# lschoenm/MerKurio

Measured on AMD Instinct MI355X. Metric: Gbases/s scanned (150bp FASTQ, 10k 31-mers); % HBM roofline at 1/2/4/8 GPUs, higher is better.
Workload: dtype u8

## Files before the change

### merkurio_amd/csrc/codec/bgzf_inflate_wave.hip

```cpp
#include <hip/hip_runtime.h>

#include "codec_kernels.h"
#include "inflate_wave_common.hpp"

namespace mkz {

namespace {

template <uint32_t kRing>
struct WaveLds {
    uint8_t ring[kRing];
    uint16_t ll_fast[1 << kFastLl];
    uint32_t d_fast[1 << kFastD];
    uint16_t ll_limit[16], ll_base[16], d_limit[16], d_base[16];
    uint16_t ll_sorted[288], d_sorted[32];
    uint8_t lens[320];
};
static_assert(sizeof(WaveLds<32768>) <= 40 * 1024, "four waves per CU");
static_assert(sizeof(WaveLds<8192>) <= 14 * 1024, "eleven waves per CU");
static_assert(sizeof(WaveLds<4096>) <= 9728, "seventeen waves per CU");

}

template <uint32_t kRing>
__global__ __launch_bounds__(64) void mk_bgzf_inflate_wave_kernel(const uint8_t *__restrict__ in_all, uint64_t n_in_all, const Member *__restrict__ members,
                                                                  uint32_t n_members, uint8_t *__restrict__ out_all, int32_t *__restrict__ status_out) {
    constexpr uint32_t kFlush = kRing >= 8192 ? 4096u : kRing / 2;
    static_assert(kRing >= 2 * kFlush && kFlush >= 1024 && (kRing & (kRing - 1)) == 0, "ring: a power of two that holds two flush pieces");
    constexpr uint32_t kRingMask = kRing - 1;
    extern __shared__ uint8_t lds_raw[];
    WaveLds<kRing> &S = *reinterpret_cast<WaveLds<kRing> *>(lds_raw);
    const uint32_t lane = lane_id();
    const uint32_t mi = blockIdx.x;
    if (mi >= n_members) return;
    const Member m = members[mi];
    const uint8_t *in = in_all + m.data_off;
    const uint32_t n_in = m.data_len, n_out = m.isize;
    uint8_t *const out = out_all + m.out_off;

    uint32_t s0 = 0, sbase = 0, rd = 0;
    uint32_t look = 0, nxt = 0;
    uint64_t bitbuf = 0;
    uint32_t bitcnt = 0;
    auto load_dword = [&](uint32_t dw) -> uint32_t {
        const uint32_t byte = s0 + 4 * dw;
        return byte <= n_in + 8 ? load_le32(in + byte) : 0u;
    };
    auto restart = [&](uint32_t byte_pos) {
        s0 = byte_pos, sbase = 0, rd = 0, bitbuf = 0, bitcnt = 0;
        look = load_dword(lane);
        nxt = load_dword(64 + lane);
    };
#define MKW_NEED32()                                                                              \
    do {                                                                                          \
        if (bitcnt < 32) {                                                                        \
            uint32_t k_ = uni(rd - sbase);                                                        \
            if (k_ == 64) {                                                                       \
                look = nxt, sbase += 64, k_ = 0;                                                  \
                nxt = load_dword(sbase + 64 + lane);                                              \
            }                                                                                     \
            bitbuf |= (uint64_t)(uint32_t)__builtin_amdgcn_readlane((int)look, (int)k_) << bitcnt; \
            bitcnt += 32, ++rd;                                                                   \
        }                                                                                         \
    } while (0)
#define MKW_TAKE(n) (bitbuf >>= (n), bitcnt -= (n))
#define MKW_TAKEN() (s0 + 4 * rd)
#define MKW_RAN_OUT() (MKW_TAKEN() > n_in + 8)
    restart(0);

    uint32_t op = 0, flushed = 0;
    int status = 0;
    auto flush_blocks = [&]() {
        while (op - flushed >= kFlush) {
#pragma unroll
            for (uint32_t k = 0; k < kFlush; k += 1024) {
                const uint32_t at = flushed + k + 16 * lane;
                const uint4 v = *reinterpret_cast<const uint4 *>(&S.ring[at & kRingMask]);
                __builtin_memcpy(out + at, &v, 16);
            }
            flushed += kFlush;
        }
        if (kRing < 32768) {
            __builtin_amdgcn_fence(__ATOMIC_RELEASE, "workgroup");
            __builtin_amdgcn_s_waitcnt(0x0F70);
        }
    };

    for (bool last_block = false; !last_block && status == 0;) {
        MKW_NEED32();
        if (MKW_RAN_OUT()) {
            status = kInfTruncated;
            break;
        }
        last_block = ((uint32_t)bitbuf & 1u) != 0;
        const uint32_t type = ((uint32_t)bitbuf >> 1) & 3u;
        MKW_TAKE(3);
        if (type == 3) {
            status = kInfBadBlockType;
            break;
        }
        if (type == 0) {
            MKW_TAKE(bitcnt & 7);
            MKW_NEED32();
            const uint32_t len = (uint32_t)bitbuf & 0xffffu, nlen = ((uint32_t)(bitbuf >> 16)) & 0xffffu;
            MKW_TAKE(32);
            const uint32_t pos = MKW_TAKEN() - (bitcnt >> 3);
            if ((len ^ nlen) != 0xffffu) status = kInfBadStored;
            else if (MKW_RAN_OUT() || pos > n_in || len > n_in - pos) status = kInfTruncated;
            else if (len > n_out - op) status = kInfOutputOverrun;
            if (status) break;
            for (uint32_t done = 0; done < len;) {
                const uint32_t piece = min(len - done, kFlush);
                for (uint32_t i = lane; i < piece; i += 64) S.ring[(op + i) & kRingMask] = in[pos + done + i];
                op += piece, done += piece;
                flush_blocks();
            }
            restart(pos + len);
            continue;
        }
        if (type == 1) {
            for (uint32_t i = lane; i < 320; i += 64) S.lens[i] = (uint8_t)(i < 144 ? 8 : i < 256 ? 9 : i < 280 ? 7 : i < 288 ? 8 : 5);
        } else {
            const uint32_t hlit = ((uint32_t)bitbuf & 31u) + 257, hdist = ((uint32_t)(bitbuf >> 5) & 31u) + 1, hclen = ((uint32_t)(bitbuf >> 10) & 15u) + 4;
            MKW_TAKE(14);
            if (hlit > 286 || hdist > 30) {
                status = kInfBadLengths;
                break;
            }
            if (lane < (uint32_t)kCl) S.lens[lane] = 0;
            constexpr uint64_t kOrderLo = 16ull | 17ull << 5 | 18ull << 10 | 0ull << 15 | 8ull << 20 | 7ull << 25 | 9ull << 30 | 6ull << 35 | 10ull << 40 |
                                          5ull << 45 | 11ull << 50 | 4ull << 55;
            constexpr uint64_t kOrderHi = 12ull | 3ull << 5 | 13ull << 10 | 2ull << 15 | 14ull << 20 | 1ull << 25 | 15ull << 30;
            for (uint32_t i = 0; i < hclen; ++i) {
                MKW_NEED32();
                const uint32_t sym = (uint32_t)((i < 12 ? kOrderLo >> (5 * i) : kOrderHi >> (5 * (i - 12))) & 31u);
                if (lane == 0) S.lens[sym] = (uint8_t)((uint32_t)bitbuf & 7u);
                MKW_TAKE(3);
            }
            if (wave_build_tables(S.lens, kCl, S.ll_sorted, S.ll_limit, S.ll_base, false)) {
                status = kInfBadLengths;
                break;
            }
            uint32_t i = 0, prev_len = 0;
            while (i < hlit + hdist && status == 0) {
                MKW_NEED32();
                if (MKW_RAN_OUT()) {
                    status = kInfTruncated;
                    break;
                }
                const uint32_t e = decode_codeword((uint32_t)bitbuf, S.ll_sorted, S.ll_limit, S.ll_base);
                if (e == 0 || (e & 15u) > (uint32_t)kMaxClBits) {
                    status = kInfBadLengths;
                    break;
                }
                MKW_TAKE(e & 15u);
                const uint32_t sym = e >> 4;
                if (sym < 16) {
                    if (lane == 0) S.lens[i < hlit ? i : 288 + (i - hlit)] = (uint8_t)sym;
                    prev_len = sym, ++i;
                    continue;
                }
                uint32_t rep, val = 0;
                if (sym == 16) {
                    if (i == 0) {
                        status = kInfBadLengths;
                        break;
                    }
                    val = prev_len;
                    rep = 3 + ((uint32_t)bitbuf & 3u);
                    MKW_TAKE(2);
                } else if (sym == 17) {
                    rep = 3 + ((uint32_t)bitbuf & 7u);
                    MKW_TAKE(3);
                } else {
                    rep = 11 + ((uint32_t)bitbuf & 127u);
                    MKW_TAKE(7);
                }
                if (i + rep > hlit + hdist) {
                    status = kInfBadLengths;
                    break;
                }
                if (lane < rep) {
                    const uint32_t j = i + lane;
                    S.lens[j < hlit ? j : 288 + (j - hlit)] = (uint8_t)val;
                }
                if (lane + 64 < rep) {
                    const uint32_t j = i + lane + 64;
                    S.lens[j < hlit ? j : 288 + (j - hlit)] = (uint8_t)val;
                }
                if (lane + 128 < rep) {
                    const uint32_t j = i + lane + 128;
                    S.lens[j < hlit ? j : 288 + (j - hlit)] = (uint8_t)val;
                }
                prev_len = val, i += rep;
            }
            if (status) break;
            for (uint32_t k = hlit + lane; k < 288; k += 64) S.lens[k] = 0;
            if (lane + hdist < 32) S.lens[288 + hdist + lane] = 0;
            __builtin_amdgcn_wave_barrier();
            if (S.lens[256] == 0) {
                status = kInfBadLengths;
                break;
            }
        }
        __builtin_amdgcn_wave_barrier();
        if (wave_build_tables(S.lens, 288, S.ll_sorted, S.ll_limit, S.ll_base, true) ||
            wave_build_tables(S.lens + 288, type == 1 ? 32 : 30, S.d_sorted, S.d_limit, S.d_base, true)) {
            status = kInfBadLengths;
            break;
        }
        __builtin_amdgcn_wave_barrier();
        wave_fill_fast_ll(S.ll_fast, S.ll_sorted, S.ll_limit, S.ll_base);
        wave_fill_fast_d(S.d_fast, S.d_sorted, S.d_limit, S.d_base);
        __builtin_amdgcn_wave_barrier();

        uint32_t flush_at = flushed + kFlush;
        for (;;) {
            MKW_NEED32();
            uint32_t e = S.ll_fast[(uint32_t)bitbuf & ((1u << kFastLl) - 1)];
            if (e == 0) {
                e = pack_ll(decode_codeword((uint32_t)bitbuf, S.ll_sorted, S.ll_limit, S.ll_base));
                if (e == 0) {
                    status = kInfBadSymbol;
                    break;
                }
            }
            MKW_TAKE(e & 15u);
            if (e < 0x1000u) {
                S.ring[op & kRingMask] = (uint8_t)(e >> 4);
                ++op;
                if (op < flush_at) continue;
            } else if (e < 0x8000u) {
                break;
            } else {
                const uint32_t leb = (e >> 4) & 7u;
                const uint32_t len = ((e >> 7) & 255u) + 3u + ((uint32_t)bitbuf & ((1u << leb) - 1));
                MKW_TAKE(leb);
                MKW_NEED32();
                uint32_t d = S.d_fast[(uint32_t)bitbuf & ((1u << kFastD) - 1)];
                if (d == 0) {
                    d = pack_d(decode_codeword((uint32_t)bitbuf, S.d_sorted, S.d_limit, S.d_base));
                    if (d == 0) {
                        status = kInfBadSymbol;
                        break;
                    }
                }
                MKW_TAKE(d & 15u);
                const uint32_t deb = (d >> 4) & 15u;
                const uint32_t dist = (d >> 8) + ((uint32_t)bitbuf & ((1u << deb) - 1));
                MKW_TAKE(deb);
                if (dist > op) {
                    status = kInfBadDistance;
                    break;
                }
                const uint32_t src0 = op - dist;
                if (kRing < 32768 && dist + len > kRing) {
                    for (uint32_t i = lane; i < len; i += 64) {
                        const uint32_t p = src0 + i;
                        const uint8_t b = p < flushed ? __hip_atomic_load(out + p, __ATOMIC_RELAXED, __HIP_MEMORY_SCOPE_AGENT) : S.ring[p & kRingMask];
                        S.ring[(op + i) & kRingMask] = b;
                    }
                } else if (dist >= len) {
                    for (uint32_t i = lane; i < len; i += 64) S.ring[(op + i) & kRingMask] = S.ring[(src0 + i) & kRingMask];
                } else {
                    for (uint32_t i = lane; i < len; i += 64) S.ring[(op + i) & kRingMask] = S.ring[(src0 + i % dist) & kRingMask];
                }
                op += len;
                if (op < flush_at) continue;
            }
            if (op > n_out) {
                status = kInfOutputOverrun;
                break;
            }
            if (MKW_RAN_OUT()) {
                status = kInfTruncated;
                break;
            }
            flush_blocks();
            flush_at = flushed + kFlush;
        }
        if (status == 0 && op > n_out) status = kInfOutputOverrun;
        if (status == 0 && MKW_RAN_OUT()) status = kInfTruncated;
    }
    if (status == 0 && (MKW_RAN_OUT() || (uint64_t)MKW_TAKEN() - (bitcnt >> 3) > (uint64_t)n_in)) status = kInfTruncated;
    if (status == 0 && op != n_out) status = kInfOutputShort;
    if (status == 0) {
        flush_blocks();
        for (uint32_t i = flushed + lane; i < op; i += 64) out[i] = S.ring[i & kRingMask];
    }
    if (lane == 0) status_out[mi] = status;
#undef MKW_NEED32
#undef MKW_TAKE
#undef MKW_TAKEN
#undef MKW_RAN_OUT
}

template <uint32_t kRing>
static void launch_ring(const uint8_t *in, uint64_t n_in, const Member *members, uint32_t n_members, uint8_t *out, int32_t *status, hipStream_t s) {
    static bool raised = false;
    if (!raised) {
        (void)hipFuncSetAttribute((const void *)mk_bgzf_inflate_wave_kernel<kRing>, hipFuncAttributeMaxDynamicSharedMemorySize, (int)sizeof(WaveLds<kRing>));
        raised = true;
    }
    hipLaunchKernelGGL(mk_bgzf_inflate_wave_kernel<kRing>, dim3(n_members), dim3(64), sizeof(WaveLds<kRing>), s, in, n_in, members, n_members, out, status);
}

void launch_inflate_wave(const uint8_t *in, uint64_t n_in, const Member *members, uint32_t n_members, uint8_t *out, int32_t *status, hipStream_t s,
                         uint32_t ring_bytes) {
    if (!n_members) return;
    if (ring_bytes == 2048) launch_ring<2048>(in, n_in, members, n_members, out, status, s);
    else if (ring_bytes == 4096) launch_ring<4096>(in, n_in, members, n_members, out, status, s);
    else if (ring_bytes == 8192) launch_ring<8192>(in, n_in, members, n_members, out, status, s);
    else if (ring_bytes == 16384) launch_ring<16384>(in, n_in, members, n_members, out, status, s);
    else launch_ring<32768>(in, n_in, members, n_members, out, status, s);
}

}
```

### merkurio_amd/csrc/codec/gzip_segments_wave.hpp

```cpp
#pragma once
#include <hip/hip_runtime.h>

#include <type_traits>

#include "gzip_segments.hpp"
#include "inflate_wave_common.hpp"

namespace mkz {
namespace {

#ifndef MK_SEG_PAIRS
#define MK_SEG_PAIRS 0
#endif
constexpr bool kSegPairs = MK_SEG_PAIRS != 0;
#ifndef MK_SEG_RING
#define MK_SEG_RING 2048
#endif
constexpr uint32_t kSegRing = MK_SEG_RING, kSegRingMask = kSegRing - 1, kSegFlush = kSegRing / 2;
constexpr uint64_t kSegCapMax = 0xfff00000ull;
constexpr int kSegCutShort = 1;
constexpr uint64_t kSegConfirmSymbols = 2048;

struct SegWaveTables {
    std::conditional_t<kSegPairs, uint32_t, uint16_t> ll_fast[1 << kFastLl];
    uint32_t d_fast[1 << kFastD];
    uint16_t ll_limit[16], ll_base[16], d_limit[16], d_base[16];
    uint16_t ll_sorted[288], d_sorted[32];
    uint8_t lens[320];
};
static_assert(kSegRing != 2048 || sizeof(SegWaveTables) + 2 * kSegRing <= (kSegPairs ? 11648 : 9728), "fourteen (without pairs: seventeen) waves per CU");
static_assert(kSegRing >= 1024 && (kSegRing & (kSegRing - 1)) == 0, "the flush writes 512 symbols a step");

template <bool kDry>
__device__ __forceinline__ int wave_inflate_segment(const uint8_t *__restrict__ in, uint64_t n_in, uint64_t bit0, uint64_t bit_end, uint32_t max_blocks,
                                    uint16_t *__restrict__ out, uint64_t cap, uint16_t *ring, SegWaveTables &S, uint64_t max_symbols, uint64_t *n_out,
                                    uint64_t *bit_stop, bool *final_seen) {
    const uint32_t lane = lane_id();
    uint64_t s0 = 0;
    uint32_t sbase = 0, rd = 0;
    uint32_t look = 0, nxt = 0;
    uint64_t bitbuf = 0;
    uint32_t bitcnt = 0;
    auto load_dword = [&](uint32_t dw) -> uint32_t {
        const uint64_t byte = s0 + 4ull * dw;
        return byte <= n_in + 8 ? load_le32(in + byte) : 0u;
    };
    auto restart = [&](uint64_t byte_pos) {
        s0 = byte_pos, sbase = 0, rd = 0, bitbuf = 0, bitcnt = 0;
        look = load_dword(lane);
        nxt = load_dword(64 + lane);
    };
#define MKS_NEED32()                                                                              \
    do {                                                                                          \
        if (bitcnt < 32) {                                                                        \
            uint32_t k_ = uni(rd - sbase);                                                        \
            if (k_ == 64) {                                                                       \
                look = nxt, sbase += 64, k_ = 0;                                                  \
                nxt = load_dword(sbase + 64 + lane);                                              \
            }                                                                                     \
            bitbuf |= (uint64_t)(uint32_t)__builtin_amdgcn_readlane((int)look, (int)k_) << bitcnt; \
            bitcnt += 32, ++rd;                                                                   \
        }                                                                                         \
    } while (0)
#define MKS_TAKE(n) (bitbuf >>= (n), bitcnt -= (n))
#define MKS_BITPOS() ((s0 + 4ull * rd) * 8 - bitcnt)
#define MKS_RAN_OUT() (MKS_BITPOS() > n_in * 8)
    restart(bit0 >> 3);
    MKS_NEED32();
    MKS_TAKE((uint32_t)bit0 & 7u);

    uint32_t op = 0, flushed = 0;
    const uint32_t cap32 = (uint32_t)(cap < kSegCapMax ? cap : kSegCapMax);
    int status = 0;
    bool fin = false;
    auto flush_blocks = [&]() {
        while (op - flushed >= kSegFlush) {
            if constexpr (!kDry) {
#pragma unroll
                for (uint32_t k = 0; k < kSegFlush; k += 512) {
                    const uint32_t at = flushed + k + 8 * lane;
                    const uint4 v = *reinterpret_cast<const uint4 *>(&ring[at & kSegRingMask]);
                    __builtin_memcpy(out + at, &v, 16);
                }
            }
            flushed += kSegFlush;
        }
        if constexpr (!kDry) {
            __builtin_amdgcn_fence(__ATOMIC_RELEASE, "workgroup");
            __builtin_amdgcn_s_waitcnt(0x0F70);
        }
    };

    for (uint32_t blocks = 0;; ++blocks) {
        const uint64_t at = MKS_BITPOS();
        if (at == bit_end || (max_blocks && blocks == max_blocks)) break;
        if (at > bit_end) {
            status = kSegDesync;
            break;
        }
        MKS_NEED32();
        if (MKS_RAN_OUT()) {
            status = kInfTruncated;
            break;
        }
        const bool final_block = ((uint32_t)bitbuf & 1u) != 0;
        const uint32_t type = ((uint32_t)bitbuf >> 1) & 3u;
        MKS_TAKE(3);
        if (type == 3) {
            status = kInfBadBlockType;
            break;
        }
        if (type == 0) {
            MKS_TAKE(bitcnt & 7);
            MKS_NEED32();
            const uint32_t len = (uint32_t)bitbuf & 0xffffu, nlen = ((uint32_t)(bitbuf >> 16)) & 0xffffu;
            MKS_TAKE(32);
            const uint64_t pos = MKS_BITPOS() >> 3;
            if ((len ^ nlen) != 0xffffu) status = kInfBadStored;
            else if (MKS_RAN_OUT() || pos > n_in || len > n_in - pos) status = kInfTruncated;
            else if (len > cap32 - op) status = kSegOverflow;
            if (status) break;
            for (uint32_t done = 0; done < len;) {
                const uint32_t piece = min(len - done, kSegFlush);
                if constexpr (!kDry)
                    for (uint32_t i = lane; i < piece; i += 64) ring[(op + i) & kSegRingMask] = in[pos + done + i];
                op += piece, done += piece;
                flush_blocks();
            }
            restart(pos + len);
        } else {
            if (type == 1) {
                for (uint32_t i = lane; i < 320; i += 64) S.lens[i] = (uint8_t)(i < 144 ? 8 : i < 256 ? 9 : i < 280 ? 7 : i < 288 ? 8 : 5);
            } else {
                const uint32_t hlit = ((uint32_t)bitbuf & 31u) + 257, hdist = ((uint32_t)(bitbuf >> 5) & 31u) + 1, hclen = ((uint32_t)(bitbuf >> 10) & 15u) + 4;
                MKS_TAKE(14);
                if (hlit > 286 || hdist > 30) {
                    status = kInfBadLengths;
                    break;
                }
                if (lane < (uint32_t)kCl) S.lens[lane] = 0;
                constexpr uint64_t kOrderLo = 16ull | 17ull << 5 | 18ull << 10 | 0ull << 15 | 8ull << 20 | 7ull << 25 | 9ull << 30 | 6ull << 35 | 10ull << 40 |
                                              5ull << 45 | 11ull << 50 | 4ull << 55;
                constexpr uint64_t kOrderHi = 12ull | 3ull << 5 | 13ull << 10 | 2ull << 15 | 14ull << 20 | 1ull << 25 | 15ull << 30;
                for (uint32_t i = 0; i < hclen; ++i) {
                    MKS_NEED32();
                    const uint32_t s_ = (uint32_t)((i < 12 ? kOrderLo >> (5 * i) : kOrderHi >> (5 * (i - 12))) & 31u);
                    if (lane == 0) S.lens[s_] = (uint8_t)((uint32_t)bitbuf & 7u);
                    MKS_TAKE(3);
                }
                if (wave_build_tables(S.lens, kCl, S.ll_sorted, S.ll_limit, S.ll_base, false)) {
                    status = kInfBadLengths;
                    break;
                }
                uint32_t i = 0, prev_len = 0;
                while (i < hlit + hdist && status == 0) {
                    MKS_NEED32();
                    if (MKS_RAN_OUT()) {
                        status = kInfTruncated;
                        break;
                    }
                    const uint32_t e = decode_codeword((uint32_t)bitbuf, S.ll_sorted, S.ll_limit, S.ll_base);
                    if (e == 0 || (e & 15u) > (uint32_t)kMaxClBits) {
                        status = kInfBadLengths;
                        break;
                    }
                    MKS_TAKE(e & 15u);
                    const uint32_t cs = e >> 4;
                    if (cs < 16) {
                        if (lane == 0) S.lens[i < hlit ? i : 288 + (i - hlit)] = (uint8_t)cs;
                        prev_len = cs, ++i;
                        continue;
                    }
                    uint32_t rep, val = 0;
                    if (cs == 16) {
                        if (i == 0) {
                            status = kInfBadLengths;
                            break;
                        }
                        val = prev_len;
                        rep = 3 + ((uint32_t)bitbuf & 3u);
                        MKS_TAKE(2);
                    } else if (cs == 17) {
                        rep = 3 + ((uint32_t)bitbuf & 7u);
                        MKS_TAKE(3);
                    } else {
                        rep = 11 + ((uint32_t)bitbuf & 127u);
                        MKS_TAKE(7);
                    }
                    if (i + rep > hlit + hdist) {
                        status = kInfBadLengths;
                        break;
                    }
                    for (uint32_t q = lane; q < rep; q += 64) {
                        const uint32_t x = i + q;
                        S.lens[x < hlit ? x : 288 + (x - hlit)] = (uint8_t)val;
                    }
                    prev_len = val, i += rep;
                }
                if (status) break;
                for (uint32_t k = hlit + lane; k < 288; k += 64) S.lens[k] = 0;
                if (lane + hdist < 32) S.lens[288 + hdist + lane] = 0;
                __builtin_amdgcn_wave_barrier();
                if (S.lens[256] == 0) {
                    status = kInfBadLengths;
                    break;
                }
            }
            __builtin_amdgcn_wave_barrier();
            if (wave_build_tables(S.lens, 288, S.ll_sorted, S.ll_limit, S.ll_base, true) ||
                wave_build_tables(S.lens + 288, type == 1 ? 32 : 30, S.d_sorted, S.d_limit, S.d_base, true)) {
                status = kInfBadLengths;
                break;
            }
            __builtin_amdgcn_wave_barrier();
            for (uint32_t e = lane; e < (1u << kFastLl); e += 64) {
                const uint32_t r = decode_codeword(e, S.ll_sorted, S.ll_limit, S.ll_base);
                S.ll_fast[e] = (r & 15u) <= (uint32_t)kFastLl ? pack_ll(r) : 0u;
            }
            __builtin_amdgcn_wave_barrier();
            if constexpr (kSegPairs) {
                for (uint32_t e = lane; e < (1u << kFastLl); e += 64) {
                    const uint32_t a = reinterpret_cast<const uint16_t *>(S.ll_fast)[2 * e];
                    const uint32_t la = a & 15u;
                    if (a != 0 && a < 0x1000u && la < (uint32_t)kFastLl) {
                        const uint32_t b = reinterpret_cast<const uint16_t *>(S.ll_fast)[2 * (e >> la)];
                        if (b != 0 && b < 0x1000u && la + (b & 15u) <= (uint32_t)kFastLl) reinterpret_cast<uint16_t *>(S.ll_fast)[2 * e + 1] = (uint16_t)((b & 0xff0u) | (la + (b & 15u)));
                    }
                }
            }
            wave_fill_fast_d(S.d_fast, S.d_sorted, S.d_limit, S.d_base);
            __builtin_amdgcn_wave_barrier();

            uint32_t flush_at = flushed + kSegFlush;
            for (;;) {
                MKS_NEED32();
                uint32_t e = S.ll_fast[(uint32_t)bitbuf & ((1u << kFastLl) - 1)];
                if (kSegPairs && e > 0xffffu) {
                    if constexpr (!kDry) {
                        ring[op & kSegRingMask] = (uint16_t)((e >> 4) & 0xffu);
                        ring[(op + 1) & kSegRingMask] = (uint16_t)(e >> 20);
                    }
                    MKS_TAKE((e >> 16) & 15u);
                    op += 2;
                    if (op < flush_at) continue;
                    e = 0x10000u;
                } else if (e == 0) {
                    e = pack_ll(decode_codeword((uint32_t)bitbuf, S.ll_sorted, S.ll_limit, S.ll_base));
                    if (e == 0) {
                        status = kInfBadSymbol;
                        break;
                    }
                }
                if (e != 0x10000u) {
                    MKS_TAKE(e & 15u);
                    if (e < 0x1000u) {
                        if constexpr (!kDry) ring[op & kSegRingMask] = (uint16_t)(e >> 4);
                        ++op;
                        if (op < flush_at) continue;
                    } else if (e < 0x8000u) {
                        break;
                    } else {
                        const uint32_t leb = (e >> 4) & 7u;
                        const uint32_t len = ((e >> 7) & 255u) + 3u + ((uint32_t)bitbuf & ((1u << leb) - 1));
                        MKS_TAKE(leb);
                        MKS_NEED32();
                        uint32_t d = S.d_fast[(uint32_t)bitbuf & ((1u << kFastD) - 1)];
                        if (d == 0) {
                            d = pack_d(decode_codeword((uint32_t)bitbuf, S.d_sorted, S.d_limit, S.d_base));
                            if (d == 0) {
                                status = kInfBadSymbol;
                                break;
                            }
                        }
                        MKS_TAKE(d & 15u);
                        const uint32_t deb = (d >> 4) & 15u;
                        const uint32_t dist = (d >> 8) + ((uint32_t)bitbuf & ((1u << deb) - 1));
                        MKS_TAKE(deb);
                        if constexpr (!kDry) {
                            const uint32_t src0 = op - dist;
                            if (dist + len > kSegRing || dist > op) {
                                for (uint32_t i = lane; i < len; i += 64) {
                                    const long long p = (long long)op - (long long)dist + (dist >= len ? i : i % dist);
                                    const uint16_t v = p < (long long)flushed ? __hip_atomic_load(out + p, __ATOMIC_RELAXED, __HIP_MEMORY_SCOPE_AGENT)
                                                                               : ring[(uint64_t)p & kSegRingMask];
                                    ring[(op + i) & kSegRingMask] = v;
                                }
                            } else if (dist >= len) {
                                for (uint32_t i = lane; i < len; i += 64) ring[(op + i) & kSegRingMask] = ring[(src0 + i) & kSegRingMask];
                            } else {
                                for (uint32_t i = lane; i < len; i += 64) ring[(op + i) & kSegRingMask] = ring[(src0 + i % dist) & kSegRingMask];
                            }
                        }
                        op += len;
                        if (op < flush_at) continue;
                    }
                }
                if (op > cap32) {
                    status = kSegOverflow;
                    break;
                }
                if (MKS_RAN_OUT()) {
                    status = kInfTruncated;
                    break;
                }
                if constexpr (kDry) {
                    if (max_symbols && op >= max_symbols) {
                        status = kSegCutShort;
                        break;
                    }
                }
                flush_blocks();
                flush_at = flushed + kSegFlush;
            }
            if (status == 0 && op > cap32) status = kSegOverflow;
            if (status == 0 && MKS_RAN_OUT()) status = kInfTruncated;
            if (status) break;
        }
        if (final_block) {
            fin = true;
            break;
        }
    }
    if constexpr (!kDry) {
        if (status == 0) {
            flush_blocks();
            for (uint32_t i = flushed + lane; i < op; i += 64) out[i] = ring[i & kSegRingMask];
        }
    }
    *n_out = op;
    *bit_stop = MKS_BITPOS();
    *final_seen = fin;
    return status;
#undef MKS_NEED32
#undef MKS_TAKE
#undef MKS_BITPOS
#undef MKS_RAN_OUT
}

__device__ __forceinline__ bool wave_confirm_block_start(const uint8_t *__restrict__ in, uint64_t n_in, uint64_t bit, SegWaveTables &S) {
    uint64_t n_out = 0, stop = 0;
    bool fin = false;
    const int rc = wave_inflate_segment<true>(in, n_in, bit, ~0ull, 1, nullptr, ~0ull, nullptr, S, kSegConfirmSymbols, &n_out, &stop, &fin);
    if (rc == kSegCutShort) return true;
    if (rc != 0) return false;
    if (n_out == 0 || fin) return false;
    if (stop + 3 > n_in * 8) return false;
    SegReader r;
    r.in = in, r.n_in = n_in;
    sr_seek(r, stop);
    const uint32_t type = ((uint32_t)r.bitbuf >> 1) & 3u;
    if (type == 2) {
        sr_take(r, 3);
        return seg_dynamic_header(r, nullptr) == 0;
    }
    if (type == 0) {
        sr_take(r, 3);
        sr_take(r, r.bitcnt & 7);
        sr_need32(r);
        const uint32_t len = (uint32_t)r.bitbuf & 0xffffu, nlen = ((uint32_t)(r.bitbuf >> 16)) & 0xffffu;
        return (len ^ nlen) == 0xffffu;
    }
    return false;
}

}
}
```

### merkurio_amd/csrc/codec/inflate_wave_common.hpp

```cpp
#pragma once
#include <hip/hip_runtime.h>

#include "inflate_serial.hpp"

namespace mkz {
namespace {

constexpr int kFastLl = 10, kFastD = 9;

__device__ __forceinline__ uint32_t lane_id() { return __builtin_amdgcn_mbcnt_hi(~0u, __builtin_amdgcn_mbcnt_lo(~0u, 0u)); }
__device__ __forceinline__ uint32_t uni(uint32_t v) { return (uint32_t)__builtin_amdgcn_readfirstlane((int)v); }

__device__ int wave_build_tables(const uint8_t *lens, uint32_t n, uint16_t *sorted, uint16_t *limit, uint16_t *base, bool allow_single) {
    const uint32_t lane = lane_id();
    uint32_t cnt = 0, used = 0;
    for (uint32_t i = 0; i < n; ++i) {
        const uint32_t v = lens[i];
        cnt += (v == lane);
        used += (v != 0);
    }
    if (lane == 0 || lane > (uint32_t)kMaxBits) cnt = 0;
    int left = 1;
    uint32_t code = 0, off = 0, my_off = 0, prev = 0;
    bool over = false;
    if (lane == 0) limit[0] = 0, base[0] = 0;
    for (uint32_t l = 1; l <= (uint32_t)kMaxBits; ++l) {
        const uint32_t c = (uint32_t)__builtin_amdgcn_readlane((int)cnt, (int)l);
        left = (left << 1) - (int)c;
        over = over || left < 0;
        code = (code + prev) << 1;
        if (lane == l) {
            my_off = off;
            limit[l] = (uint16_t)((code + c) << (kMaxBits - l));
            base[l] = (uint16_t)(off - code);
        }
        off += c;
        prev = c;
    }
    if (over) return 1;
    for (uint32_t c0 = 0; c0 < n; c0 += 64) {
        const uint32_t i = c0 + lane;
        const uint32_t mine = i < n ? lens[i] : 0u;
        for (uint32_t l = 1; l <= (uint32_t)kMaxBits; ++l) {
            const uint64_t m = __ballot(mine == l);
            if (m == 0) continue;
            const uint32_t o = (uint32_t)__builtin_amdgcn_readlane((int)my_off, (int)l);
            if (mine == l) sorted[o + (uint32_t)__popcll(m & ((1ull << lane) - 1))] = (uint16_t)i;
            if (lane == l) my_off += (uint32_t)__popcll(m);
        }
    }
    const uint32_t c1 = (uint32_t)__builtin_amdgcn_readlane((int)cnt, 1);
    if (left > 0 && !(used == 0 || (allow_single && used == 1 && c1 == 1))) return 2;
    return 0;
}

__device__ __forceinline__ uint32_t pack_ll(uint32_t r) {
    const uint32_t sym = r >> 4;
    if (sym <= 256) return r;
    if (sym > 285) return 0;
    const uint32_t idx = sym - 257;
    return 0x8000u | (length_base(idx) - 3) << 7 | length_extra_bits(idx) << 4 | (r & 15u);
}
__device__ __forceinline__ uint32_t pack_d(uint32_t r) {
    const uint32_t sym = r >> 4;
    if (r == 0 || sym > 29) return 0;
    return distance_base(sym) << 8 | distance_extra_bits(sym) << 4 | (r & 15u);
}
__device__ void wave_fill_fast_ll(uint16_t *fast, const uint16_t *sorted, const uint16_t *limit, const uint16_t *base) {
    for (uint32_t e = lane_id(); e < (1u << kFastLl); e += 64) {
        const uint32_t r = decode_codeword(e, sorted, limit, base);
        fast[e] = (uint16_t)((r & 15u) <= (uint32_t)kFastLl ? pack_ll(r) : 0u);
    }
}
__device__ void wave_fill_fast_d(uint32_t *fast, const uint16_t *sorted, const uint16_t *limit, const uint16_t *base) {
    for (uint32_t e = lane_id(); e < (1u << kFastD); e += 64) {
        const uint32_t r = decode_codeword(e, sorted, limit, base);
        fast[e] = (r & 15u) <= (uint32_t)kFastD ? pack_d(r) : 0u;
    }
}


}
}
```

Measured before the change: 6241.

## Restructure wave inflate bitstream and match copy for branchless uniform decoding

Moves the duplicated bit-reader logic into a shared WaveStream helper. The helper uses a clamped load and a precomputed end index, so the bounds check becomes a select and the window advances after the readlane instead of before it. Fast-table lookups go through readfirstlane so values stay scalar. Near match copies write the first 64 lanes unconditionally, sending lanes past the match length to a dump area, and replace the integer modulo for overlapping matches with a reciprocal-float approximation. The literal/length loop is flattened into one branchy-light loop with a run flag and expect hints, and the code-length fill is unrolled to a fixed 192 trip count. The float modulo trick and dump writes into the lens scratch carry correctness risk.

```diff
diff --git a/merkurio_amd/csrc/codec/bgzf_inflate_wave.hip b/merkurio_amd/csrc/codec/bgzf_inflate_wave.hip
--- a/merkurio_amd/csrc/codec/bgzf_inflate_wave.hip
+++ b/merkurio_amd/csrc/codec/bgzf_inflate_wave.hip
@@ -38,35 +38,12 @@
     const uint32_t n_in = m.data_len, n_out = m.isize;
     uint8_t *const out = out_all + m.out_off;
 
-    uint32_t s0 = 0, sbase = 0, rd = 0;
-    uint32_t look = 0, nxt = 0;
-    uint64_t bitbuf = 0;
-    uint32_t bitcnt = 0;
-    auto load_dword = [&](uint32_t dw) -> uint32_t {
-        const uint32_t byte = s0 + 4 * dw;
-        return byte <= n_in + 8 ? load_le32(in + byte) : 0u;
-    };
-    auto restart = [&](uint32_t byte_pos) {
-        s0 = byte_pos, sbase = 0, rd = 0, bitbuf = 0, bitcnt = 0;
-        look = load_dword(lane);
-        nxt = load_dword(64 + lane);
-    };
-#define MKW_NEED32()                                                                              \
-    do {                                                                                          \
-        if (bitcnt < 32) {                                                                        \
-            uint32_t k_ = uni(rd - sbase);                                                        \
-            if (k_ == 64) {                                                                       \
-                look = nxt, sbase += 64, k_ = 0;                                                  \
-                nxt = load_dword(sbase + 64 + lane);                                              \
-            }                                                                                     \
-            bitbuf |= (uint64_t)(uint32_t)__builtin_amdgcn_readlane((int)look, (int)k_) << bitcnt; \
-            bitcnt += 32, ++rd;                                                                   \
-        }                                                                                         \
-    } while (0)
-#define MKW_TAKE(n) (bitbuf >>= (n), bitcnt -= (n))
-#define MKW_TAKEN() (s0 + 4 * rd)
+    WaveStream<uint32_t> st;
+    ws_init(st, in, n_in, 0u);
+#define MKW_NEED32() ws_need32(st)
+#define MKW_TAKE(n) ws_take(st, (n))
+#define MKW_TAKEN() ws_taken(st)
 #define MKW_RAN_OUT() (MKW_TAKEN() > n_in + 8)
-    restart(0);
 
     uint32_t op = 0, flushed = 0;
     int status = 0;
@@ -92,19 +69,19 @@
             status = kInfTruncated;
             break;
         }
-        last_block = ((uint32_t)bitbuf & 1u) != 0;
-        const uint32_t type = ((uint32_t)bitbuf >> 1) & 3u;
+        last_block = ((uint32_t)st.bitbuf & 1u) != 0;
+        const uint32_t type = ((uint32_t)st.bitbuf >> 1) & 3u;
         MKW_TAKE(3);
         if (type == 3) {
             status = kInfBadBlockType;
             break;
         }
         if (type == 0) {
-            MKW_TAKE(bitcnt & 7);
+            MKW_TAKE(st.bitcnt & 7);
             MKW_NEED32();
-            const uint32_t len = (uint32_t)bitbuf & 0xffffu, nlen = ((uint32_t)(bitbuf >> 16)) & 0xffffu;
+            const uint32_t len = (uint32_t)st.bitbuf & 0xffffu, nlen = ((uint32_t)(st.bitbuf >> 16)) & 0xffffu;
             MKW_TAKE(32);
-            const uint32_t pos = MKW_TAKEN() - (bitcnt >> 3);
+            const uint32_t pos = MKW_TAKEN() - (st.bitcnt >> 3);
             if ((len ^ nlen) != 0xffffu) status = kInfBadStored;
             else if (MKW_RAN_OUT() || pos > n_in || len > n_in - pos) status = kInfTruncated;
             else if (len > n_out - op) status = kInfOutputOverrun;
@@ -115,13 +92,13 @@
                 op += piece, done += piece;
                 flush_blocks();
             }
-            restart(pos + len);
+            ws_restart(st, pos + len);
             continue;
         }
         if (type == 1) {
             for (uint32_t i = lane; i < 320; i += 64) S.lens[i] = (uint8_t)(i < 144 ? 8 : i < 256 ? 9 : i < 280 ? 7 : i < 288 ? 8 : 5);
         } else {
-            const uint32_t hlit = ((uint32_t)bitbuf & 31u) + 257, hdist = ((uint32_t)(bitbuf >> 5) & 31u) + 1, hclen = ((uint32_t)(bitbuf >> 10) & 15u) + 4;
+            const uint32_t hlit = ((uint32_t)st.bitbuf & 31u) + 257, hdist = ((uint32_t)(st.bitbuf >> 5) & 31u) + 1, hclen = ((uint32_t)(st.bitbuf >> 10) & 15u) + 4;
             MKW_TAKE(14);
             if (hlit > 286 || hdist > 30) {
                 status = kInfBadLengths;
@@ -134,7 +111,7 @@
             for (uint32_t i = 0; i < hclen; ++i) {
                 MKW_NEED32();
                 const uint32_t sym = (uint32_t)((i < 12 ? kOrderLo >> (5 * i) : kOrderHi >> (5 * (i - 12))) & 31u);
-                if (lane == 0) S.lens[sym] = (uint8_t)((uint32_t)bitbuf & 7u);
+                if (lane == 0) S.lens[sym] = (uint8_t)((uint32_t)st.bitbuf & 7u);
                 MKW_TAKE(3);
             }
             if (wave_build_tables(S.lens, kCl, S.ll_sorted, S.ll_limit, S.ll_base, false)) {
@@ -148,7 +125,7 @@
                     status = kInfTruncated;
                     break;
                 }
-                const uint32_t e = decode_codeword((uint32_t)bitbuf, S.ll_sorted, S.ll_limit, S.ll_base);
+                const uint32_t e = decode_codeword((uint32_t)st.bitbuf, S.ll_sorted, S.ll_limit, S.ll_base);
                 if (e == 0 || (e & 15u) > (uint32_t)kMaxClBits) {
                     status = kInfBadLengths;
                     break;
@@ -167,13 +144,13 @@
                         break;
                     }
                     val = prev_len;
-                    rep = 3 + ((uint32_t)bitbuf & 3u);
+                    rep = 3 + ((uint32_t)st.bitbuf & 3u);
                     MKW_TAKE(2);
                 } else if (sym == 17) {
-                    rep = 3 + ((uint32_t)bitbuf & 7u);
+                    rep = 3 + ((uint32_t)st.bitbuf & 7u);
                     MKW_TAKE(3);
                 } else {
-                    rep = 11 + ((uint32_t)bitbuf & 127u);
+                    rep = 11 + ((uint32_t)st.bitbuf & 127u);
                     MKW_TAKE(7);
                 }
                 if (i + rep > hlit + hdist) {
@@ -215,74 +192,60 @@
         __builtin_amdgcn_wave_barrier();
 
         uint32_t flush_at = flushed + kFlush;
-        for (;;) {
+        for (bool run = true; run;) {
             MKW_NEED32();
-            uint32_t e = S.ll_fast[(uint32_t)bitbuf & ((1u << kFastLl) - 1)];
-            if (e == 0) {
-                e = pack_ll(decode_codeword((uint32_t)bitbuf, S.ll_sorted, S.ll_limit, S.ll_base));
-                if (e == 0) {
-                    status = kInfBadSymbol;
-                    break;
-                }
+            uint32_t e = wave_fast(S.ll_fast, (uint32_t)st.bitbuf & ((1u << kFastLl) - 1));
+            if (__builtin_expect(e == 0, 0)) {
+                e = pack_ll(decode_codeword((uint32_t)st.bitbuf, S.ll_sorted, S.ll_limit, S.ll_base));
+                if (e == 0) status = kInfBadSymbol, e = 0x1000u;
             }
             MKW_TAKE(e & 15u);
             if (e < 0x1000u) {
                 S.ring[op & kRingMask] = (uint8_t)(e >> 4);
                 ++op;
-                if (op < flush_at) continue;
-            } else if (e < 0x8000u) {
-                break;
-            } else {
+            } else if (e >= 0x8000u) {
                 const uint32_t leb = (e >> 4) & 7u;
-                const uint32_t len = ((e >> 7) & 255u) + 3u + ((uint32_t)bitbuf & ((1u << leb) - 1));
+                const uint32_t len = ((e >> 7) & 255u) + 3u + ((uint32_t)st.bitbuf & ((1u << leb) - 1));
                 MKW_TAKE(leb);
                 MKW_NEED32();
-                uint32_t d = S.d_fast[(uint32_t)bitbuf & ((1u << kFastD) - 1)];
-                if (d == 0) {
-                    d = pack_d(decode_codeword((uint32_t)bitbuf, S.d_sorted, S.d_limit, S.d_base));
-                    if (d == 0) {
-                        status = kInfBadSymbol;
-                        break;
-                    }
-                }
+                uint32_t d = wave_fast(S.d_fast, (uint32_t)st.bitbuf & ((1u << kFastD) - 1));
+                if (__builtin_expect(d == 0, 0)) d = pack_d(decode_codeword((uint32_t)st.bitbuf, S.d_sorted, S.d_limit, S.d_base));
                 MKW_TAKE(d & 15u);
                 const uint32_t deb = (d >> 4) & 15u;
-                const uint32_t dist = (d >> 8) + ((uint32_t)bitbuf & ((1u << deb) - 1));
+                const uint32_t dist = (d >> 8) + ((uint32_t)st.bitbuf & ((1u << deb) - 1));
                 MKW_TAKE(deb);
-                if (dist > op) {
-                    status = kInfBadDistance;
-                    break;
-                }
-                const uint32_t src0 = op - dist;
-                if (kRing < 32768 && dist + len > kRing) {
+                if (__builtin_expect(d == 0 || dist > op, 0)) {
+                    status = d == 0 ? kInfBadSymbol : kInfBadDistance;
+                    run = false;
+                } else if (kRing < 32768 && dist + len > kRing) {
+                    const uint32_t src0 = op - dist;
                     for (uint32_t i = lane; i < len; i += 64) {
                         const uint32_t p = src0 + i;
                         const uint8_t b = p < flushed ? __hip_atomic_load(out + p, __ATOMIC_RELAXED, __HIP_MEMORY_SCOPE_AGENT) : S.ring[p & kRingMask];
                         S.ring[(op + i) & kRingMask] = b;
                     }
-                } else if (dist >= len) {
-                    for (uint32_t i = lane; i < len; i += 64) S.ring[(op + i) & kRingMask] = S.ring[(src0 + i) & kRingMask];
+                    op += len;
                 } else {
-                    for (uint32_t i = lane; i < len; i += 64) S.ring[(op + i) & kRingMask] = S.ring[(src0 + i % dist) & kRingMask];
-                }
-                op += len;
-                if (op < flush_at) continue;
-            }
-            if (op > n_out) {
-                status = kInfOutputOverrun;
-                break;
-            }
-            if (MKW_RAN_OUT()) {
-                status = kInfTruncated;
-                break;
-            }
-            flush_blocks();
-            flush_at = flushed + kFlush;
-        }
+                    wave_copy_near<kRingMask>(S.ring, S.lens, op, dist, len);
+                    op += len;
+                }
+            } else {
+                run = false;
+            }
+            if (__builtin_expect(run && op >= flush_at, 0)) {
+                if (op > n_out) status = kInfOutputOverrun, run = false;
+                else if (MKW_RAN_OUT()) status = kInfTruncated, run = false;
+                else {
+                    flush_blocks();
+                    flush_at = flushed + kFlush;
+                }
+            }
+        }
+        if (status) break;
         if (status == 0 && op > n_out) status = kInfOutputOverrun;
         if (status == 0 && MKW_RAN_OUT()) status = kInfTruncated;
     }
-    if (status == 0 && (MKW_RAN_OUT() || (uint64_t)MKW_TAKEN() - (bitcnt >> 3) > (uint64_t)n_in)) status = kInfTruncated;
+    if (status == 0 && (MKW_RAN_OUT() || (uint64_t)MKW_TAKEN() - (st.bitcnt >> 3) > (uint64_t)n_in)) status = kInfTruncated;
     if (status == 0 && op != n_out) status = kInfOutputShort;
     if (status == 0) {
         flush_blocks();
diff --git a/merkurio_amd/csrc/codec/gzip_segments_wave.hpp b/merkurio_amd/csrc/codec/gzip_segments_wave.hpp
--- a/merkurio_amd/csrc/codec/gzip_segments_wave.hpp
+++ b/merkurio_amd/csrc/codec/gzip_segments_wave.hpp
@@ -36,36 +36,12 @@
                                     uint16_t *__restrict__ out, uint64_t cap, uint16_t *ring, SegWaveTables &S, uint64_t max_symbols, uint64_t *n_out,
                                     uint64_t *bit_stop, bool *final_seen) {
     const uint32_t lane = lane_id();
-    uint64_t s0 = 0;
-    uint32_t sbase = 0, rd = 0;
-    uint32_t look = 0, nxt = 0;
-    uint64_t bitbuf = 0;
-    uint32_t bitcnt = 0;
-    auto load_dword = [&](uint32_t dw) -> uint32_t {
-        const uint64_t byte = s0 + 4ull * dw;
-        return byte <= n_in + 8 ? load_le32(in + byte) : 0u;
-    };
-    auto restart = [&](uint64_t byte_pos) {
-        s0 = byte_pos, sbase = 0, rd = 0, bitbuf = 0, bitcnt = 0;
-        look = load_dword(lane);
-        nxt = load_dword(64 + lane);
-    };
-#define MKS_NEED32()                                                                              \
-    do {                                                                                          \
-        if (bitcnt < 32) {                                                                        \
-            uint32_t k_ = uni(rd - sbase);                                                        \
-            if (k_ == 64) {                                                                       \
-                look = nxt, sbase += 64, k_ = 0;                                                  \
-                nxt = load_dword(sbase + 64 + lane);                                              \
-            }                                                                                     \
-            bitbuf |= (uint64_t)(uint32_t)__builtin_amdgcn_readlane((int)look, (int)k_) << bitcnt; \
-            bitcnt += 32, ++rd;                                                                   \
-        }                                                                                         \
-    } while (0)
-#define MKS_TAKE(n) (bitbuf >>= (n), bitcnt -= (n))
-#define MKS_BITPOS() ((s0 + 4ull * rd) * 8 - bitcnt)
+    WaveStream<uint64_t> st;
+    ws_init(st, in, n_in, bit0 >> 3);
+#define MKS_NEED32() ws_need32(st)
+#define MKS_TAKE(n) ws_take(st, (n))
+#define MKS_BITPOS() (ws_taken(st) * 8 - st.bitcnt)
 #define MKS_RAN_OUT() (MKS_BITPOS() > n_in * 8)
-    restart(bit0 >> 3);
     MKS_NEED32();
     MKS_TAKE((uint32_t)bit0 & 7u);
 
@@ -103,17 +79,17 @@
             status = kInfTruncated;
             break;
         }
-        const bool final_block = ((uint32_t)bitbuf & 1u) != 0;
-        const uint32_t type = ((uint32_t)bitbuf >> 1) & 3u;
+        const bool final_block = ((uint32_t)st.bitbuf & 1u) != 0;
+        const uint32_t type = ((uint32_t)st.bitbuf >> 1) & 3u;
         MKS_TAKE(3);
         if (type == 3) {
             status = kInfBadBlockType;
             break;
         }
         if (type == 0) {
-            MKS_TAKE(bitcnt & 7);
+            MKS_TAKE(st.bitcnt & 7);
             MKS_NEED32();
-            const uint32_t len = (uint32_t)bitbuf & 0xffffu, nlen = ((uint32_t)(bitbuf >> 16)) & 0xffffu;
+            const uint32_t len = (uint32_t)st.bitbuf & 0xffffu, nlen = ((uint32_t)(st.bitbuf >> 16)) & 0xffffu;
             MKS_TAKE(32);
             const uint64_t pos = MKS_BITPOS() >> 3;
             if ((len ^ nlen) != 0xffffu) status = kInfBadStored;
@@ -127,12 +103,12 @@
                 op += piece, done += piece;
                 flush_blocks();
             }
-            restart(pos + len);
+            ws_restart(st, pos + len);
         } else {
             if (type == 1) {
                 for (uint32_t i = lane; i < 320; i += 64) S.lens[i] = (uint8_t)(i < 144 ? 8 : i < 256 ? 9 : i < 280 ? 7 : i < 288 ? 8 : 5);
             } else {
-                const uint32_t hlit = ((uint32_t)bitbuf & 31u) + 257, hdist = ((uint32_t)(bitbuf >> 5) & 31u) + 1, hclen = ((uint32_t)(bitbuf >> 10) & 15u) + 4;
+                const uint32_t hlit = ((uint32_t)st.bitbuf & 31u) + 257, hdist = ((uint32_t)(st.bitbuf >> 5) & 31u) + 1, hclen = ((uint32_t)(st.bitbuf >> 10) & 15u) + 4;
                 MKS_TAKE(14);
                 if (hlit > 286 || hdist > 30) {
                     status = kInfBadLengths;
@@ -145,7 +121,7 @@
                 for (uint32_t i = 0; i < hclen; ++i) {
                     MKS_NEED32();
                     const uint32_t s_ = (uint32_t)((i < 12 ? kOrderLo >> (5 * i) : kOrderHi >> (5 * (i - 12))) & 31u);
-                    if (lane == 0) S.lens[s_] = (uint8_t)((uint32_t)bitbuf & 7u);
+                    if (lane == 0) S.lens[s_] = (uint8_t)((uint32_t)st.bitbuf & 7u);
                     MKS_TAKE(3);
                 }
                 if (wave_build_tables(S.lens, kCl, S.ll_sorted, S.ll_limit, S.ll_base, false)) {
@@ -159,7 +135,7 @@
                         status = kInfTruncated;
                         break;
                     }
-                    const uint32_t e = decode_codeword((uint32_t)bitbuf, S.ll_sorted, S.ll_limit, S.ll_base);
+                    const uint32_t e = decode_codeword((uint32_t)st.bitbuf, S.ll_sorted, S.ll_limit, S.ll_base);
                     if (e == 0 || (e & 15u) > (uint32_t)kMaxClBits) {
                         status = kInfBadLengths;
                         break;
@@ -178,22 +154,23 @@
                             break;
                         }
                         val = prev_len;
-                        rep = 3 + ((uint32_t)bitbuf & 3u);
+                        rep = 3 + ((uint32_t)st.bitbuf & 3u);
                         MKS_TAKE(2);
                     } else if (cs == 17) {
-                        rep = 3 + ((uint32_t)bitbuf & 7u);
+                        rep = 3 + ((uint32_t)st.bitbuf & 7u);
                         MKS_TAKE(3);
                     } else {
-                        rep = 11 + ((uint32_t)bitbuf & 127u);
+                        rep = 11 + ((uint32_t)st.bitbuf & 127u);
                         MKS_TAKE(7);
                     }
                     if (i + rep > hlit + hdist) {
                         status = kInfBadLengths;
                         break;
                     }
-                    for (uint32_t q = lane; q < rep; q += 64) {
+#pragma unroll
+                    for (uint32_t q = lane; q < 192; q += 64) {
                         const uint32_t x = i + q;
-                        S.lens[x < hlit ? x : 288 + (x - hlit)] = (uint8_t)val;
+                        if (q < rep) S.lens[x < hlit ? x : 288 + (x - hlit)] = (uint8_t)val;
                     }
                     prev_len = val, i += rep;
                 }
@@ -234,7 +211,7 @@
             uint32_t flush_at = flushed + kSegFlush;
             for (;;) {
                 MKS_NEED32();
-                uint32_t e = S.ll_fast[(uint32_t)bitbuf & ((1u << kFastLl) - 1)];
+                uint32_t e = wave_fast(S.ll_fast, (uint32_t)st.bitbuf & ((1u << kFastLl) - 1));
                 if (kSegPairs && e > 0xffffu) {
                     if constexpr (!kDry) {
                         ring[op & kSegRingMask] = (uint16_t)((e >> 4) & 0xffu);
@@ -244,8 +221,8 @@
                     op += 2;
                     if (op < flush_at) continue;
                     e = 0x10000u;
-                } else if (e == 0) {
-                    e = pack_ll(decode_codeword((uint32_t)bitbuf, S.ll_sorted, S.ll_limit, S.ll_base));
+                } else if (__builtin_expect(e == 0, 0)) {
+                    e = pack_ll(decode_codeword((uint32_t)st.bitbuf, S.ll_sorted, S.ll_limit, S.ll_base));
                     if (e == 0) {
                         status = kInfBadSymbol;
                         break;
@@ -261,12 +238,12 @@
                         break;
                     } else {
                         const uint32_t leb = (e >> 4) & 7u;
-                        const uint32_t len = ((e >> 7) & 255u) + 3u + ((uint32_t)bitbuf & ((1u << leb) - 1));
+                        const uint32_t len = ((e >> 7) & 255u) + 3u + ((uint32_t)st.bitbuf & ((1u << leb) - 1));
                         MKS_TAKE(leb);
                         MKS_NEED32();
-                        uint32_t d = S.d_fast[(uint32_t)bitbuf & ((1u << kFastD) - 1)];
-                        if (d == 0) {
-                            d = pack_d(decode_codeword((uint32_t)bitbuf, S.d_sorted, S.d_limit, S.d_base));
+                        uint32_t d = wave_fast(S.d_fast, (uint32_t)st.bitbuf & ((1u << kFastD) - 1));
+                        if (__builtin_expect(d == 0, 0)) {
+                            d = pack_d(decode_codeword((uint32_t)st.bitbuf, S.d_sorted, S.d_limit, S.d_base));
                             if (d == 0) {
                                 status = kInfBadSymbol;
                                 break;
@@ -274,10 +251,9 @@
                         }
                         MKS_TAKE(d & 15u);
                         const uint32_t deb = (d >> 4) & 15u;
-                        const uint32_t dist = (d >> 8) + ((uint32_t)bitbuf & ((1u << deb) - 1));
+                        const uint32_t dist = (d >> 8) + ((uint32_t)st.bitbuf & ((1u << deb) - 1));
                         MKS_TAKE(deb);
                         if constexpr (!kDry) {
-                            const uint32_t src0 = op - dist;
                             if (dist + len > kSegRing || dist > op) {
                                 for (uint32_t i = lane; i < len; i += 64) {
                                     const long long p = (long long)op - (long long)dist + (dist >= len ? i : i % dist);
@@ -285,10 +261,8 @@
                                                                                : ring[(uint64_t)p & kSegRingMask];
                                     ring[(op + i) & kSegRingMask] = v;
                                 }
-                            } else if (dist >= len) {
-                                for (uint32_t i = lane; i < len; i += 64) ring[(op + i) & kSegRingMask] = ring[(src0 + i) & kSegRingMask];
                             } else {
-                                for (uint32_t i = lane; i < len; i += 64) ring[(op + i) & kSegRingMask] = ring[(src0 + i % dist) & kSegRingMask];
+                                wave_copy_near<kSegRingMask>(ring, reinterpret_cast<uint16_t *>(S.lens), op, dist, len);
                             }
                         }
                         op += len;
diff --git a/merkurio_amd/csrc/codec/inflate_wave_common.hpp b/merkurio_amd/csrc/codec/inflate_wave_common.hpp
--- a/merkurio_amd/csrc/codec/inflate_wave_common.hpp
+++ b/merkurio_amd/csrc/codec/inflate_wave_common.hpp
@@ -24,6 +24,7 @@
     uint32_t code = 0, off = 0, my_off = 0, prev = 0;
     bool over = false;
     if (lane == 0) limit[0] = 0, base[0] = 0;
+#pragma unroll 1
     for (uint32_t l = 1; l <= (uint32_t)kMaxBits; ++l) {
         const uint32_t c = (uint32_t)__builtin_amdgcn_readlane((int)cnt, (int)l);
         left = (left << 1) - (int)c;
@@ -41,6 +42,7 @@
     for (uint32_t c0 = 0; c0 < n; c0 += 64) {
         const uint32_t i = c0 + lane;
         const uint32_t mine = i < n ? lens[i] : 0u;
+#pragma unroll 1
         for (uint32_t l = 1; l <= (uint32_t)kMaxBits; ++l) {
             const uint64_t m = __ballot(mine == l);
             if (m == 0) continue;
@@ -79,6 +81,83 @@
     }
 }
 
+template <typename Pos>
+struct WaveStream {
+    const uint8_t *in;
+    Pos s0;
+    Pos lim;
+    uint32_t rd;
+    uint32_t rd_end;
+    uint32_t look, nxt;
+    uint64_t bitbuf;
+    uint32_t bitcnt;
+};
+
+template <typename Pos>
+__device__ __forceinline__ uint32_t ws_load(const WaveStream<Pos> &s, uint32_t dw) {
+    const Pos b = s.s0 + (Pos)4 * dw;
+    return load_le32(s.in + (b < s.lim ? b : s.lim));
+}
+template <typename Pos>
+__device__ __forceinline__ void ws_restart(WaveStream<Pos> &s, Pos byte_pos) {
+    const uint32_t lane = lane_id();
+    s.s0 = byte_pos, s.rd = 0, s.bitbuf = 0, s.bitcnt = 0;
+    const Pos room = byte_pos <= s.lim ? (s.lim - byte_pos) / 4 + 1 : 0;
+    s.rd_end = room < (Pos)0xffffffffu ? (uint32_t)room : 0xffffffffu;
+    s.look = ws_load(s, lane);
+    s.nxt = ws_load(s, 64 + lane);
+}
+template <typename Pos>
+__device__ __forceinline__ void ws_init(WaveStream<Pos> &s, const uint8_t *in, Pos n_in, Pos byte_pos) {
+    s.in = in, s.lim = n_in + 8;
+    ws_restart(s, byte_pos);
+}
+template <typename Pos>
+__device__ __forceinline__ void ws_need32(WaveStream<Pos> &s) {
+    if (s.bitcnt < 32) {
+        uint32_t w = (uint32_t)__builtin_amdgcn_readlane((int)s.look, (int)(s.rd & 63u));
+        w = s.rd < s.rd_end ? w : 0u;
+        s.bitbuf |= (uint64_t)w << s.bitcnt;
+        s.bitcnt += 32, ++s.rd;
+        if ((s.rd & 63u) == 0) {
+            s.look = s.nxt;
+            s.nxt = ws_load(s, s.rd + 64 + lane_id());
+        }
+    }
+}
+template <typename Pos>
+__device__ __forceinline__ void ws_take(WaveStream<Pos> &s, uint32_t n) {
+    s.bitbuf >>= n, s.bitcnt -= n;
+}
+template <typename Pos>
+__device__ __forceinline__ Pos ws_taken(const WaveStream<Pos> &s) {
+    return s.s0 + (Pos)4 * s.rd;
+}
+
+template <typename T>
+__device__ __forceinline__ uint32_t wave_fast(const T *fast, uint32_t idx) {
+    return uni((uint32_t)fast[idx]);
+}
+
+template <uint32_t kMask, typename T>
+__device__ __forceinline__ void wave_copy_near(T *ring, T *dump, uint32_t op, uint32_t dist, uint32_t len) {
+    const uint32_t lane = lane_id();
+    const uint32_t src0 = op - dist;
+    if (dist >= len) {
+        const T v = ring[(src0 + lane) & kMask];
+        *(lane < len ? &ring[(op + lane) & kMask] : &dump[lane]) = v;
+        if (len > 64)
+            for (uint32_t i = 64 + lane; i < len; i += 64) ring[(op + i) & kMask] = ring[(src0 + i) & kMask];
+    } else {
+        const float r = __builtin_amdgcn_rcpf((float)dist);
+        auto mod = [&](uint32_t i) { return i - (uint32_t)__builtin_fmaf((float)i, r, 1.0f / 512) * dist; };
+        const T v = ring[(src0 + mod(lane)) & kMask];
+        *(lane < len ? &ring[(op + lane) & kMask] : &dump[lane]) = v;
+        if (len > 64)
+            for (uint32_t i = 64 + lane; i < len; i += 64) ring[(op + i) & kMask] = ring[(src0 + mod(i)) & kMask];
+    }
+}
+
 
 }
 }
```

New measurement: 6240 (median of 5 runs). Within noise of the previous version (-0.0%).
